# mcgill-cpslab/all-pairs-similarity

Hardware: AMD Instinct MI355X
Metric: scored candidate pairs/sec + achieved HBM GB/s, N=1M d=100k nnz=100, 1/2/4/8 GPU (higher is better)
Workload: dtype u16+f32

## Files before the change

### all-pairs-similarity_amd/csrc/apss_even.hpp

```cpp
#pragma once
#include <type_traits>
#include "apss_kernels.hpp"

namespace apss {

using ProbeArgsK = const __attribute__((address_space(4))) ProbeArgs;

template <int BLOCK, int U, int LONGCAP, bool SHARD, bool SIGNED, bool ACC8, bool MERGE, bool TWO = false>
__device__ __forceinline__ void probe_even_item(ProbeArgsK &a, const int tile, const int v0, const int v1, const bool own_tile, const bool first) {
  constexpr int NW = BLOCK / kWave;
  static_assert(NW == 8 || NW == 16, "8 or 16 waves");
  constexpr int NS = NW - 1;
  constexpr bool SLOT2 = BLOCK <= 512;
  constexpr uint32_t ABITS = ACC8 ? 8u : 16u;
  constexpr bool WIDE = ACC8 && BLOCK > 512;
  constexpr int CH = 16, LPC = CH / 2, GPW = kWave / LPC, WIN = GPW * U;
  constexpr int SLOTS = 2 * WIN < 48 ? 2 * WIN : (WIN > 48 ? WIN : 48);
  static_assert(SLOTS >= WIN, "the register window reads the first WIN slots of a strip");
  constexpr int GS = BLOCK > 512 ? SLOTS / GPW : ((SLOTS / GPW) + 1) & ~1;
  constexpr int SSZ = GPW * GS;
  static_assert(GPW == 8 && SLOTS % GPW == 0, "slot <-> (step, group) by shifts");
  constexpr int kLongLen = kLongLenW;
  constexpr int CBMAX = WIDE ? 131072 : (BLOCK <= 512 && !ACC8 ? 32768 : 65536);
  constexpr int APW = 32 / (int)ABITS;
  constexpr bool LEAN = !SIGNED;
  static_assert(1 + (NW - 1) * 2 * U < (1 << (ACC8 ? 8 : 16)), "the spare words' low accumulators must not wrap within a round");
  static_assert(!TWO || (BLOCK == 512 && ACC8 && !MERGE && !SIGNED && !SHARD), "two planes: the plain 512-thread kernel, 8-bit sums");
  __shared__ __attribute__((aligned(16))) uint32_t acc[CBMAX / APW + kWave];
  __shared__ __attribute__((aligned(16))) uint2 strips[3 * NS * SSZ + kWave];
  __shared__ uint2 longs[3 * LONGCAP];
  __shared__ float long_w[3 * LONGCAP];
  __shared__ uint2 facts[4];
  __shared__ unsigned long long stat[4];
  unsigned char *const smem_raw = reinterpret_cast<unsigned char *>(acc);
  uint32_t *const facts_w = reinterpret_cast<uint32_t *>(facts);

  int tid = threadIdx.x;
  asm volatile("" : "+v"(tid));
  const int wv = __builtin_amdgcn_readfirstlane(tid / kWave), ln = tid % kWave;
  const int cb = a.cb;
  const int F = a.flat_waves;
  const int A = NW - F;
  const int CAP = A * SLOTS;
  const uint32_t A8 = (uint32_t)A * (uint32_t)GPW;
  const float rcpA8 = 1.0f / (float)A8;
  const uint32_t magicA8 = 0xffffffffu / A8 + 1u;
  const int LOGG = a.flat_group_log2, G = 1 << LOGG;
  const uint32_t sub = (uint32_t)ln & (uint32_t)(G - 1);
  static_assert(!MERGE || SHARD, "merged rounds: term shards only");
  const int mlaunch = MERGE ? a.merge_log2 : 0;
  const int mlog = own_tile ? 0 : mlaunch;
  const int nv = own_tile ? a.nq_rows : a.nq;
  const int qtile = (v0 << mlog) / cb;
  const int64_t tile_row0 = (int64_t)tile * cb;
  const int unmerged_mark = own_tile ? kUnmergedBit : 0;
  const uint32_t lo = (uint32_t)(ln % LPC);
  const float cxs = a.cx_scale;

  const int64_t qbase = uniform_load(a.q_rowptr + (MERGE ? min(v0 << mlog, a.nq_rows) : v0)), qend = uniform_load(a.q_rowptr + (MERGE ? min(v1 << mlog, a.nq_rows) : v1));
  const int64_t pbase = uniform_load(a.tile_post_base + tile), pend = uniform_load(a.tile_post_base + tile + 1);
  const __amdgpu_buffer_rsrc_t rs_qi =
      __builtin_amdgcn_make_buffer_rsrc((void *)(a.q_idx + qbase), 0, (int)((qend - qbase) * 4), 0x00020000);
  const __amdgpu_buffer_rsrc_t rs_qv =
      __builtin_amdgcn_make_buffer_rsrc((void *)(a.q_val + qbase), 0, (int)((qend - qbase) * 4), 0x00020000);
  const __amdgpu_buffer_rsrc_t rs_tp = __builtin_amdgcn_make_buffer_rsrc(
      (void *)(a.tile_seg + (int64_t)tile * a.seg_stride), 0, (int)(a.seg_stride * 8), 0x00020000);
  const __amdgpu_buffer_rsrc_t rs_po =
      __builtin_amdgcn_make_buffer_rsrc((void *)(a.post_c + pbase), 0, (int)((pend - pbase) * 4), 0x00020000);
  constexpr uint32_t kOob = 0xfffffff0u;
  constexpr uint32_t kStale = 0x80000000u, kSwept = 0x40000000u;
  constexpr uint32_t kRare = 0x80000000u;
  constexpr uint32_t kCountMask = 0xffffu;
  constexpr int kFirstSkippable = BLOCK > 512 || !SHARD ? U - 1 : 0;

  if (first) {
    for (int i = tid * 4; i < cb / APW; i += BLOCK * 4) *reinterpret_cast<uint4 *>(acc + i) = make_uint4(0u, 0u, 0u, 0u);
    if constexpr (TWO)
      for (int i = tid * 4; i < cb / APW; i += BLOCK * 4) *reinterpret_cast<uint4 *>(acc + cb / APW + i) = make_uint4(0u, 0u, 0u, 0u);
  }
  if (tid < kWave) acc[CBMAX / APW + tid] = 1u;
  if (LEAN) {
    for (int i = tid; i < 3 * NS * SSZ; i += BLOCK) strips[i].x = kStale;
  }
  if (tid < 8) facts_w[tid] = 0;
  unsigned long long my_visits = 0;
  uint32_t my_cands = 0;
  uint32_t n_seen = 0;

  struct RowExt { int qb; int nnz; };
  struct TermW { uint32_t term; float w, qs; bool valid; };
  struct Seg { uint32_t s, len; float w; };
  struct WaveWork {
    uint32_t info;
    uint32_t flags;
    apss_u32x2 pc[U];
    float wq[U];
  };
  const int32_t *const rowptr_lo = reinterpret_cast<const int32_t *>(a.q_rowptr);
  const int qbase_lo = (int)(uint32_t)qbase;
  auto load_R = [&](int v) {
    RowExt r;
    const int row_a = min(v, nv - 1) << mlog, row_b = MERGE ? min(row_a + (1 << mlog), a.nq_rows) : row_a + 1;
    r.qb = rowptr_lo[2 * row_a];
    r.nnz = rowptr_lo[2 * row_b];
    return r;
  };
  auto load_I = [&](const RowExt &r, const int fi, const int v) {
    TermW t;
    const int kterm = ((fi * kWave) >> LOGG) + (ln >> LOGG);
    const int nnz = v < v1 ? r.nnz - r.qb : 0;
    t.valid = kterm < nnz;
    const uint32_t off = t.valid ? (uint32_t)(r.qb - qbase_lo + kterm) * 4u : kOob;
    t.term = __builtin_amdgcn_raw_buffer_load_b32(rs_qi, off, 0, 0);
    t.w = __uint_as_float(__builtin_amdgcn_raw_buffer_load_b32(rs_qv, off, 0, 0));
    t.qs = SHARD && !MERGE ? a.q_scale[min(v, nv - 1)] : 1.0f;
    return t;
  };
  auto load_P = [&](const TermW &t) {
    Seg g;
    const apss_u32x2 sg = __builtin_amdgcn_raw_buffer_load_b64(rs_tp, t.valid ? t.term * 8u : kOob, 0, 0);
    g.s = sg.x;
    g.len = sg.y;
    g.w = SHARD ? (t.qs > 0.f ? t.w * __builtin_amdgcn_rcpf(t.qs) : 0.f) : t.w;
    return g;
  };
  uint2 *const spare_item = strips + 3 * NS * SSZ + ln;
  auto flatten = [&](const Seg &g, const int ring, const int fs) {
    uint32_t len = g.len;
    my_visits += sub == 0u ? len : 0u;
    const bool is_long = len > (uint32_t)kLongLen;
    len = is_long ? 0u : len;
    const uint32_t nch = (len + CH - 1) / CH;
    const uint32_t mine = sub == 0u ? nch : 0u;
    const uint32_t incl = wave_incl_scan(mine);
    uint32_t base = 0;
    if (ln == kWave - 1) base = atomicAdd(&facts_w[2 * fs], incl);
    uint32_t j0 = (uint32_t)__builtin_amdgcn_readlane((int)base, kWave - 1) + incl - mine;
    if (LOGG == 2) j0 = (uint32_t)__builtin_amdgcn_update_dpp((int)j0, (int)j0, 0x00, 0xf, 0xf, false);
    else if (LOGG == 1) j0 = (uint32_t)__builtin_amdgcn_update_dpp((int)j0, (int)j0, 0xa0, 0xf, 0xf, false);
    const uint32_t wbits = __float_as_uint(cxs * g.w);
    uint2 *const st = strips + ring * (NS * SSZ);
    auto put = [&](const uint32_t k) {
      const uint32_t j = min(j0 + k, (uint32_t)CAP - 1u);
      const uint32_t u = (uint32_t)(((float)j + 0.5f) * rcpA8);
      const uint32_t r = j - u * A8;
      uint2 *const dst = k < nch ? st + (r >> 3) * SSZ + (r & 7u) * GS + u : spare_item;
      *dst = make_uint2((g.s + k * CH) * 4u, wbits);
    };
    const uint32_t two = LOGG == 2 ? 8u : (LOGG == 1 ? 6u : 3u);
    put(sub);
    put(sub + (uint32_t)G);
    if (LOGG < 2) put(sub + 2u * (uint32_t)G);
    const bool unfit = j0 + nch > (uint32_t)CAP;
    if (__any(is_long || unfit || nch > two)) {
      bool bad = unfit;
      if (is_long && sub == 0u) {
        const uint32_t k = atomicAdd(&facts_w[2 * fs + 1], 2u) >> 1;
        if (k < (uint32_t)LONGCAP) {
          longs[ring * LONGCAP + k] = make_uint2(g.s, g.len);
          long_w[ring * LONGCAP + k] = g.w;
        } else {
          bad = true;
        }
      }
      if (bad) atomicOr(&facts_w[2 * fs + 1], 1u);
      for (uint32_t k = two + sub; __any(k < nch); k += (uint32_t)G) put(k);
    }
  };
  struct StripRead { uint2 fc; uint2 it[U]; };
  auto strip_read = [&](StripRead &sr, const int ring, const int rank, const int fs) {
    sr.fc = facts[fs];
    const uint2 *const st = strips + (ring * NS + rank) * SSZ + (ln / LPC) * GS;
    if constexpr (GS % 2 == 0) {
#pragma unroll
      for (int u = 0; u + 1 < U; u += 2) {
        const uint4 two = *reinterpret_cast<const uint4 *>(st + u);
        sr.it[u] = make_uint2(two.x, two.y);
        sr.it[u + 1] = make_uint2(two.z, two.w);
      }
      if (U & 1) sr.it[U - 1] = st[U - 1];
    } else {
#pragma unroll
      for (int u = 0; u < U; ++u) sr.it[u] = st[u];
    }
    if (LEAN) {
      uint2 *const own = strips + (ring * NS + rank) * SSZ + (ln & 7) * GS + (ln >> 3);
      (ln < WIN ? own : spare_item)->x = kStale;
    }
  };
  auto strip_loads = [&](WaveWork &f, StripRead &sr, const int rank) {
    const uint32_t fx = (uint32_t)__builtin_amdgcn_readfirstlane((int)sr.fc.x), fy = (uint32_t)__builtin_amdgcn_readfirstlane((int)sr.fc.y);
    const uint32_t tot = (fy & 1u) ? 0u : fx;
    const uint32_t full = __umulhi(tot, magicA8);
    const int rem = (int)(tot - full * A8) - GPW * rank;
    const uint32_t mine = (uint32_t)GPW * full + (uint32_t)min(max(rem, 0), GPW);
    const bool rare = fy != 0u || tot > (uint32_t)(A * WIN);
    const uint32_t steps = min(full + (rem > 0 ? 1u : 0u), (uint32_t)U);
    f.info = mine | (rare ? kRare : 0u) | (steps << 16);
    f.flags = sr.fc.y;
#pragma unroll
    for (int u = 0; u < U; ++u) asm volatile("" : "+v"(sr.it[u].x), "+v"(sr.it[u].y));
    const uint32_t lane_off = lo * 8u + (LEAN && (fy & 1u) ? kSwept : 0u);
#pragma unroll
    for (int u = 0; u < U; ++u) {
      f.wq[u] = __uint_as_float(sr.it[u].y);
      const uint32_t off = LEAN ? sr.it[u].x + lane_off : ((uint32_t)(u * GPW + ln / LPC) < mine ? sr.it[u].x + lo * 8u : kOob);
      f.pc[u] = __builtin_amdgcn_raw_buffer_load_b64(rs_po, off, 0, 0);
    }
  };

  const bool stager = wv < F;
  const int rank = wv - F;
  WaveWork wfa, wfb;
  if constexpr (TWO) {
    wfb.info = 0u;
#pragma unroll
    for (int u = 0; u < U; ++u) wfb.pc[u] = apss_u32x2{0u, 0u};
  }
  constexpr int slack = 2;
  const int thr_c = (int)a.cx_theta - slack;
  const uint32_t thr1 = (uint32_t)max(thr_c, 1) - 1u;
  {
    const TermW I0 = load_I(load_R(v0), wv, v0), I1 = load_I(load_R(v0 + 1), wv, v0 + 1);
    const Seg P0 = load_P(I0), P1 = load_P(I1);
    __syncthreads();
    if (stager) {
      flatten(P0, 0, TWO ? 3 : 0);
      flatten(P1, 1, 1);
    }
    __syncthreads();
    if (!stager) {
      StripRead sr;
      strip_read(sr, 0, rank, TWO ? 3 : 0);
      strip_loads(wfa, sr, rank);
    }
  }

  if (stager) {
    RowExt R4 = load_R(v0 + 4);
    TermW Ic = load_I(load_R(v0 + 3), wv, v0 + 3);
    Seg Pc = load_P(load_I(load_R(v0 + 2), wv, v0 + 2));
    int r0 = 0;
    for (int v = v0; v < v1; ++v) {
      const int r2 = r0 == 0 ? 2 : r0 - 1;
      const RowExt R5 = load_R(v + 5);
      const TermW In = load_I(R4, wv, v + 4);
      const Seg Pn = load_P(Ic);
      flatten(Pc, r2, r2);
      if constexpr (TWO) {
        if (tid == 0) facts[r0] = make_uint2(0u, 0u);
        __syncthreads();
      } else {
        __syncthreads();
        if (tid == 0) facts[r0] = make_uint2(0u, 0u);
        __syncthreads();
      }
      R4 = R5;
      Ic = In;
      Pc = Pn;
      r0 = r0 == 2 ? 0 : r0 + 1;
    }
  } else {
    const int atid = tid - F * kWave, ABLOCK = A * kWave;
    auto clear_round = [&](const WaveWork &w, const uint32_t P) {
      *reinterpret_cast<uint32_t *>(smem_raw + (uint32_t)(CBMAX / APW) * 4u + (uint32_t)ln * 4u) = 0x0101u;
      if ((w.info & kRare) != 0u) {
        const uint32_t keep = P ? 0x00ff00ffu : 0xff00ff00u;
        for (int i = atid; i < cb / 2; i += ABLOCK) __hip_atomic_fetch_and(acc + i, keep, __ATOMIC_RELAXED, __HIP_MEMORY_SCOPE_WORKGROUP);
      } else {
        const int n = (int)((w.info >> 16) & 0xfu);
#pragma unroll
        for (int u = 0; u < U; ++u) {
          if (u >= kFirstSkippable && u >= n) break;
          smem_raw[(w.pc[u].x & 0xffffu) + P] = 0;
          smem_raw[(w.pc[u].y & 0xffffu) + P] = 0;
        }
      }
    };
    auto round = [&](auto plane, WaveWork &w0, WaveWork &w2, const int v, const int r0) {
      constexpr uint32_t P = TWO ? (uint32_t)decltype(plane)::value : 0u;
      const int r1 = r0 == 2 ? 0 : r0 + 1;
      const int q = v;
      auto report = [&](const bool cross, const uint32_t slot, const uint32_t sum) {
        bool ok = cross;
        if (ok && mlog == 0) ok = a.ext_id[tile_row0 + slot] != a.q_ext[q];
        const uint64_t o = wave_append(ok, &a.counters[kCtrResults]);
        if (ok && o < a.res_cap) {
          a.res_q[o] = q | unmerged_mark;
          a.res_c[o] = (int32_t)(tile_row0 + slot);
          a.res_s[o] = (float)sum / cxs;
        }
      };
      auto report_lane = [&](const uint32_t slot, const uint32_t sum) {
        if (mlog != 0 || a.ext_id[tile_row0 + slot] != a.q_ext[q]) {
          const uint64_t o = atomicAdd(&a.counters[kCtrResults], 1ull);
          if (o < a.res_cap) {
            a.res_q[o] = q | unmerged_mark;
            a.res_c[o] = (int32_t)(tile_row0 + slot);
            a.res_s[o] = (float)sum / cxs;
          }
        }
      };
      auto slot_of = [&](const uint32_t pcw) { return WIDE ? pcw >> 15 : (SLOT2 && (!ACC8 || TWO) ? (pcw & 0xffffu) >> 1 : pcw & 0xffffu); };
      auto prod = [&](const uint32_t pcw, const float wqs) {
        const float x = __builtin_fmaf(wqs, __half2float(__ushort_as_half((unsigned short)(WIDE ? pcw & 0x7fffu : pcw >> 16))), 1.0f);
        return SIGNED ? (uint32_t)max((int)x, 1) : (uint32_t)x;
      };
      auto half_of = [&](const uint32_t old_word, const uint32_t pcw) {
        if (WIDE) return __builtin_amdgcn_ubfe(old_word, (pcw >> 12) & 24u, 8u);
        if (TWO) return __builtin_amdgcn_ubfe(old_word, (pcw << 3) + 8u * P, 8u);
        return SLOT2 ? __builtin_amdgcn_ubfe(old_word, pcw << 3, ABITS) : (old_word >> ((pcw & 1u) << 4)) & 0xffffu;
      };
      constexpr int BATCH = 3;
      const uint32_t spare = (uint32_t)(CBMAX / APW) * 4u + (uint32_t)ln * 4u;
      auto add_or_spare = [&](const uint32_t pcw, const uint32_t p) -> uint32_t {
        if constexpr (TWO) {
          return atomicAdd(reinterpret_cast<uint32_t *>(smem_raw + (pcw ? pcw & 0xfffcu : spare)), p << (((pcw << 3) + 8u * P) & 31u));
        }
        const uint32_t addr = WIDE ? (pcw >> 15) & 0x1fffcu : (SLOT2 ? pcw & 0xfffcu : ((pcw & 0xffffu) >> 1) * 4u);
        const uint32_t sh = WIDE ? (pcw >> 12) & 24u : (SLOT2 ? (pcw << 3) & 31u : (pcw & 1u) << 4);
        return atomicAdd(reinterpret_cast<uint32_t *>(smem_raw + (pcw ? addr : spare)), p << sh);
      };
      auto visit2 = [&](const uint32_t x, const uint32_t y, const float wqs) {
        const uint32_t px = prod(x, wqs), py = prod(y, wqs);
        uint32_t ox = add_or_spare(x, LEAN && x == 0u ? 0u : px), oy = add_or_spare(y, LEAN && y == 0u ? 0u : py);
        ox = x ? half_of(ox, x) : thr1 + 1u;
        oy = y ? half_of(oy, y) : thr1 + 1u;
        my_cands += (ox == 0u ? 1u : 0u) + (oy == 0u ? 1u : 0u);
        if ((thr1 - ox < px) | (thr1 - oy < py)) {
          if (thr1 - ox < px) report_lane(slot_of(x), ox + px);
          if (thr1 - oy < py) report_lane(slot_of(y), oy + py);
        }
      };
      const int n_steps = (int)((w0.info >> 16) & 0xfu);
      if (LEAN) n_seen -= 2u * (uint32_t)max(n_steps, kFirstSkippable);
      auto issue_batch = [&](const int u0, uint32_t (&p0)[BATCH], uint32_t (&p1)[BATCH], uint32_t (&o0)[BATCH], uint32_t (&o1)[BATCH]) {
#pragma unroll
        for (int j = 0; j < BATCH; ++j) {
          const int u = u0 + j;
          if (u >= kFirstSkippable && u >= n_steps) break;
          if (u < U) {
            p0[j] = prod(w0.pc[u].x, w0.wq[u]);
            p1[j] = prod(w0.pc[u].y, w0.wq[u]);
            o0[j] = add_or_spare(w0.pc[u].x, p0[j]);
            o1[j] = add_or_spare(w0.pc[u].y, p1[j]);
          }
        }
      };
      auto check_batch = [&](const int u0, uint32_t (&p0)[BATCH], uint32_t (&p1)[BATCH], uint32_t (&o0)[BATCH], uint32_t (&o1)[BATCH]) {
        if constexpr (LEAN) {
          uint32_t top = 0;
#pragma unroll
          for (int j = 0; j < BATCH; ++j) {
            const int u = u0 + j;
            if (u >= kFirstSkippable && u >= n_steps) break;
            if (u < U) {
              o0[j] = half_of(o0[j], w0.pc[u].x);
              o1[j] = half_of(o1[j], w0.pc[u].y);
              uint32_t s0, s1;
              asm("v_min_u32 %0, 1, %1" : "=v"(s0) : "v"(o0[j]));
              asm("v_min_u32 %0, 1, %1" : "=v"(s1) : "v"(o1[j]));
              n_seen += s0 + s1;
              top = max(max(top, o0[j] + p0[j]), o1[j] + p1[j]);
            }
          }
          if (__any(top > thr1)) {
#pragma unroll
            for (int j = 0; j < BATCH; ++j) {
              const int u = u0 + j;
              if (u >= kFirstSkippable && u >= n_steps) break;
              if (u < U) {
                const uint32_t a0 = w0.pc[u].x ? o0[j] : thr1 + 1u, a1 = w0.pc[u].y ? o1[j] : thr1 + 1u;
                report(thr1 - a0 < p0[j], slot_of(w0.pc[u].x), a0 + p0[j]);
                report(thr1 - a1 < p1[j], slot_of(w0.pc[u].y), a1 + p1[j]);
              }
            }
          }
          return;
        }
        uint32_t n_cross = 0;
#pragma unroll
        for (int j = 0; j < BATCH; ++j) {
          const int u = u0 + j;
          if (u >= kFirstSkippable && u >= n_steps) break;
          if (u < U) {
            o0[j] = w0.pc[u].x ? half_of(o0[j], w0.pc[u].x) : thr1 + 1u;
            o1[j] = w0.pc[u].y ? half_of(o1[j], w0.pc[u].y) : thr1 + 1u;
            my_cands += (o0[j] == 0u ? 1u : 0u) + (o1[j] == 0u ? 1u : 0u);
            n_cross += (thr1 - o0[j] < p0[j] ? 1u : 0u) + (thr1 - o1[j] < p1[j] ? 1u : 0u);
          }
        }
        if (__any(n_cross != 0u)) {
#pragma unroll
          for (int j = 0; j < BATCH; ++j) {
            const int u = u0 + j;
            if (u >= kFirstSkippable && u >= n_steps) break;
            if (u < U) {
              report(thr1 - o0[j] < p0[j], slot_of(w0.pc[u].x), o0[j] + p0[j]);
              report(thr1 - o1[j] < p1[j], slot_of(w0.pc[u].y), o1[j] + p1[j]);
            }
          }
        }
      };
      if constexpr (TWO) clear_round(w2, P ^ 1u);
      StripRead sr;
      strip_read(sr, r1, rank, r1);
      {
        uint32_t p0[BATCH], p1[BATCH], o0[BATCH], o1[BATCH];
        issue_batch(0, p0, p1, o0, o1);
        asm volatile("" : "+v"(sr.fc.x), "+v"(sr.fc.y) : : "memory");
        __builtin_amdgcn_sched_barrier(0);
        strip_loads(w2, sr, rank);
        check_batch(0, p0, p1, o0, o1);
      }
#pragma unroll
      for (int u0 = BATCH; u0 < U; u0 += BATCH) {
        uint32_t p0[BATCH], p1[BATCH], o0[BATCH], o1[BATCH];
        issue_batch(u0, p0, p1, o0, o1);
        check_batch(u0, p0, p1, o0, o1);
      }
      const bool rare = (w0.info & kRare) != 0u;
      if (rare) {
        const uint32_t flags = (uint32_t)__builtin_amdgcn_readfirstlane((int)w0.flags);
        const int mc = (int)(w0.info & kCountMask);
        if (mc > WIN) {
          const uint2 *const st = strips + (r0 * NS + rank) * SSZ;
          for (int c0 = WIN; c0 < mc; c0 += GPW) {
            const int c = c0 + ln / LPC;
            const int cc = min(c, SLOTS - 1);
            const uint2 it = st[(cc & 7) * GS + (cc >> 3)];
            const apss_u32x2 two = __builtin_amdgcn_raw_buffer_load_b64(rs_po, c < mc ? it.x + lo * 8u : kOob, 0, 0);
            visit2(two.x, two.y, __uint_as_float(it.y));
          }
        }
        if (flags & 1u) {
          RowExt cur = load_R(v);
          cur.nnz -= cur.qb;
          cur.qb -= qbase_lo;
          const float qsv = SHARD && !MERGE ? uniform_load(a.q_scale + v) : 1.0f;
          const float iq = qsv > 0.f ? 1.0f / qsv : 0.f;
          for (int k = rank; k < cur.nnz; k += A) {
            const uint32_t off = (uint32_t)(cur.qb + k) * 4u;
            const uint32_t term = __builtin_amdgcn_raw_buffer_load_b32(rs_qi, off, 0, 0);
            const float wq_ = cxs * __uint_as_float(__builtin_amdgcn_raw_buffer_load_b32(rs_qv, off, 0, 0)) * iq;
            const apss_u32x2 sg = __builtin_amdgcn_raw_buffer_load_b64(rs_tp, term * 8u, 0, 0);
            for (uint32_t p = 2u * (uint32_t)ln; p < sg.y; p += 2u * kWave) {
              const apss_u32x2 two = __builtin_amdgcn_raw_buffer_load_b64(rs_po, (sg.x + p) * 4u, 0, 0);
              visit2(two.x, p + 1u < sg.y ? two.y : 0u, wq_);
            }
          }
        } else {
          const uint32_t n_long = min(flags >> 1, (uint32_t)LONGCAP);
          for (uint32_t j = 0; j < n_long; ++j) {
            const uint2 sgm = longs[r0 * LONGCAP + j];
            const float wq_ = cxs * long_w[r0 * LONGCAP + j];
            for (uint32_t k = 2u * (uint32_t)atid; k < sgm.y; k += 2u * (uint32_t)ABLOCK) {
              const apss_u32x2 a0 = __builtin_amdgcn_raw_buffer_load_b64(rs_po, (sgm.x + k) * 4u, 0, 0);
              visit2(a0.x, k + 1u < sgm.y ? a0.y : 0u, wq_);
            }
          }
        }
      }
      __syncthreads();
      if constexpr (TWO) return;

      if (LEAN) *reinterpret_cast<uint32_t *>(smem_raw + spare) = 1u;
      if (rare) {
        for (int i = atid * 4; i < cb / APW; i += ABLOCK * 4) *reinterpret_cast<uint4 *>(acc + i) = make_uint4(0u, 0u, 0u, 0u);
      } else {
        unsigned short *acc16w = reinterpret_cast<unsigned short *>(acc);
#pragma unroll
        for (int u = 0; u < U; ++u) {
          if (u >= kFirstSkippable && u >= n_steps) break;
          if (WIDE) {
            smem_raw[w0.pc[u].x >> 15] = 0;
            smem_raw[w0.pc[u].y >> 15] = 0;
          } else if (SLOT2 && ACC8) {
            smem_raw[w0.pc[u].x & 0xffffu] = 0;
            smem_raw[w0.pc[u].y & 0xffffu] = 0;
          } else if (SLOT2) {
            *reinterpret_cast<unsigned short *>(smem_raw + (w0.pc[u].x & 0xffffu)) = 0;
            *reinterpret_cast<unsigned short *>(smem_raw + (w0.pc[u].y & 0xffffu)) = 0;
          } else {
            acc16w[w0.pc[u].x & 0xffffu] = 0;
            acc16w[w0.pc[u].y & 0xffffu] = 0;
          }
        }
      }
      __syncthreads();
    };
    int r0 = 0;
    constexpr std::integral_constant<int, 0> even_round{};
    constexpr std::integral_constant<int, TWO ? 1 : 0> odd_round{};
    for (int v = v0; v < v1; v += 2) {
      round(even_round, wfa, wfb, v, r0);
      r0 = r0 == 2 ? 0 : r0 + 1;
      if (v + 1 >= v1) break;
      round(odd_round, wfb, wfa, v + 1, r0);
      r0 = r0 == 2 ? 0 : r0 + 1;
    }
    if constexpr (TWO) {
      if ((v1 - v0) & 1) clear_round(wfa, 0u);
      else clear_round(wfb, 1u);
    }
  }
  __syncthreads();
  if (tid < 3) stat[tid] = 0;
  __syncthreads();
  atomicAdd(&stat[0], my_visits);
  atomicAdd(&stat[1], (unsigned long long)(my_cands - n_seen));
  __syncthreads();
  if (tid == 0) {
    const unsigned long long twice = a.tri && tile < qtile ? 2ull : 1ull;
    atomicAdd(&a.counters[kCtrVisits], stat[0] * twice);
    atomicAdd(&a.counters[kCtrCands], stat[1] * twice);
    atomicAdd(&a.counters[kCtrDevVisits], stat[0]);
  }
}

template <int BLOCK, int U, int LONGCAP, bool SHARD, bool SIGNED, bool ACC8, bool MERGE, bool TWO = false>
__device__ __forceinline__ void probe_even_body(const ProbeArgs &a) {
  int g_tile = 0, g_v0 = 0, g_v1 = 0;
  if (!a.items) {
    const int cb = a.cb, mlaunch = MERGE ? a.merge_log2 : 0;
    const int tile = a.tile0 + blockIdx.x / a.n_chunks;
    const int c0 = (blockIdx.x % a.n_chunks) * a.q_chunk;
    const int row_lo = c0 << mlaunch, row_hi = MERGE ? min(a.nq_rows, (c0 + a.q_chunk) << mlaunch) : 0;
    const bool own_tile = mlaunch != 0 && a.q_slot_base >= 0 && (a.q_slot_base + row_lo) / cb <= tile && tile <= (a.q_slot_base + row_hi - 1) / cb;
    if (a.tri && tile > row_lo / cb) return;
    g_tile = tile | (own_tile ? kUnmergedBit : 0);
    g_v0 = own_tile ? row_lo : c0;
    g_v1 = own_tile ? row_hi : min(a.nq, c0 + a.q_chunk);
    asm volatile("" : "+s"(g_tile), "+s"(g_v0), "+s"(g_v1));
  }
  __shared__ int next_item;
  for (bool first = true;; first = false) {
    int tile, v0, v1;
    bool own_tile;
    if (a.items) {
      if (threadIdx.x == 0) next_item = (int)atomicAdd(a.work_ctr, 1ull);
      __syncthreads();
      const int idx = __builtin_amdgcn_readfirstlane(next_item);
      if (idx >= a.n_items) return;
      const ProbeItem *const it = a.items + idx;
      tile = uniform_load(&it->tile);
      v0 = uniform_load(&it->v0);
      v1 = uniform_load(&it->v1);
      own_tile = uniform_load(&it->own) != 0;
    } else {
      if (!first) return;
      tile = g_tile & ~kUnmergedBit;
      v0 = g_v0;
      v1 = g_v1;
      own_tile = (g_tile & kUnmergedBit) != 0;
    }
    ProbeArgsK *ak = reinterpret_cast<ProbeArgsK *>(reinterpret_cast<uintptr_t>(__builtin_amdgcn_kernarg_segment_ptr()));
    asm volatile("" : "+s"(ak));
    probe_even_item<BLOCK, U, LONGCAP, SHARD, SIGNED, ACC8, MERGE, TWO>(*ak, tile, v0, v1, own_tile, first);
  }
}

template <int BLOCK, int U, int LONGCAP, bool SHARD, bool SIGNED, bool ACC8>
__global__ __launch_bounds__(BLOCK, BLOCK <= 512 ? 2 * BLOCK / 256 : BLOCK / 256) void k_probe_even(const ProbeArgs a) {
  probe_even_body<BLOCK, U, LONGCAP, SHARD, SIGNED, ACC8, false>(a);
}

template <int U, bool ACC8>
__global__ __launch_bounds__(512, 4) void k_probe_even_merged(const ProbeArgs a) {
  probe_even_body<512, U, 128, true, false, ACC8, true>(a);
}

template <int U>
__global__ __launch_bounds__(512, 4) void k_probe_planes(const ProbeArgs a) {
  probe_even_body<512, U, 128, false, false, true, false, true>(a);
}

}
```

Before: 1081 billion.

## Wipe idle accumulator plane with bulk ds_write_addtid instead of per-candidate clears

For the two-plane 8-bit kernel with U>=5, the accumulator planes are split into separate 32 KB LDS regions. Each wave now zeros the idle plane wholesale using ds_write_addtid_b32 through M0 while it stages or scores the other plane. This replaces the scattered per-candidate byte clears and the atomic AND sweep on rare rounds. The trade is a fixed wipe cost proportional to the accumulator size every round, plus an lgkmcnt wait before each barrier, in exchange for fewer scattered LDS stores and simpler indexing.

```diff
diff --git a/all-pairs-similarity_amd/csrc/apss_even.hpp b/all-pairs-similarity_amd/csrc/apss_even.hpp
--- a/all-pairs-similarity_amd/csrc/apss_even.hpp
+++ b/all-pairs-similarity_amd/csrc/apss_even.hpp
@@ -26,6 +26,8 @@
   constexpr bool LEAN = !SIGNED;
   static_assert(1 + (NW - 1) * 2 * U < (1 << (ACC8 ? 8 : 16)), "the spare words' low accumulators must not wrap within a round");
   static_assert(!TWO || (BLOCK == 512 && ACC8 && !MERGE && !SIGNED && !SHARD), "two planes: the plain 512-thread kernel, 8-bit sums");
+  constexpr bool WIPE = TWO && U >= 5;
+  constexpr uint32_t kPlane = 32768u;
   __shared__ __attribute__((aligned(16))) uint32_t acc[CBMAX / APW + kWave];
   __shared__ __attribute__((aligned(16))) uint2 strips[3 * NS * SSZ + kWave];
   __shared__ uint2 longs[3 * LONGCAP];
@@ -76,7 +78,7 @@
   if (first) {
     for (int i = tid * 4; i < cb / APW; i += BLOCK * 4) *reinterpret_cast<uint4 *>(acc + i) = make_uint4(0u, 0u, 0u, 0u);
     if constexpr (TWO)
-      for (int i = tid * 4; i < cb / APW; i += BLOCK * 4) *reinterpret_cast<uint4 *>(acc + cb / APW + i) = make_uint4(0u, 0u, 0u, 0u);
+      for (int i = tid * 4; i < cb / APW; i += BLOCK * 4) *reinterpret_cast<uint4 *>(acc + (WIPE ? (int)kPlane / 4 : cb / APW) + i) = make_uint4(0u, 0u, 0u, 0u);
   }
   if (tid < kWave) acc[CBMAX / APW + tid] = 1u;
   if (LEAN) {
@@ -86,6 +88,37 @@
   unsigned long long my_visits = 0;
   uint32_t my_cands = 0;
   uint32_t n_seen = 0;
+
+  static_assert(!WIPE || sizeof(strips) + sizeof(longs) + sizeof(long_w) + sizeof(facts) + sizeof(stat) + 256  + 256 * (NW - 1) < 65536,
+                "M0[15:0] must hold the LDS address of acc + 256 wv wherever acc lies");
+  const int wipe_n = WIPE ? ((cb + 255) >> 8) - wv : 0;
+  const uint32_t wipe_m0 = (uint32_t)(uintptr_t)(__attribute__((address_space(3))) uint32_t *)acc + 256u * (uint32_t)wv;
+  auto wipe = [&](auto plane_c) {
+    constexpr int PL = (int)decltype(plane_c)::value * (int)kPlane;
+    uint32_t zero = 0u;
+    asm volatile("" : "+v"(zero));
+    uint32_t keep;
+    int n = wipe_n;
+    asm volatile("" : "+s"(n));
+#define APSS_WIPE_FOUR(JB)                                                                                                        \
+  if (32 * (JB) < n)                                                                                                              \
+    asm volatile("s_mov_b32 %0, m0\n\ts_mov_b32 m0, %2\n\ts_nop 0\n\t"                                                            \
+                 "ds_write_addtid_b32 %1 offset:%3\n\tds_write_addtid_b32 %1 offset:%4\n\t"                                      \
+                 "ds_write_addtid_b32 %1 offset:%5\n\tds_write_addtid_b32 %1 offset:%6\n\t"                                      \
+                 "s_mov_b32 m0, %0"                                                                                              \
+                 : "=&s"(keep)                                                                                                   \
+                 : "v"(zero), "s"(wipe_m0), "i"(PL + 8192 * (JB)), "i"(PL + 8192 * (JB) + 2048), "i"(PL + 8192 * (JB) + 4096),   \
+                   "i"(PL + 8192 * (JB) + 6144)                                                                                  \
+                 : "memory")
+    APSS_WIPE_FOUR(0);
+    APSS_WIPE_FOUR(1);
+    APSS_WIPE_FOUR(2);
+    APSS_WIPE_FOUR(3);
+#undef APSS_WIPE_FOUR
+  };
+  constexpr std::integral_constant<int, 0> plane0{};
+  constexpr std::integral_constant<int, 1> plane1{};
+  auto wipe_wait = [&] { asm volatile("s_waitcnt lgkmcnt(0)" : : : "memory"); };
 
   struct RowExt { int qb; int nnz; };
   struct TermW { uint32_t term; float w, qs; bool valid; };
@@ -241,14 +274,21 @@
     TermW Ic = load_I(load_R(v0 + 3), wv, v0 + 3);
     Seg Pc = load_P(load_I(load_R(v0 + 2), wv, v0 + 2));
     int r0 = 0;
+    uint32_t idle = kPlane;
     for (int v = v0; v < v1; ++v) {
       const int r2 = r0 == 0 ? 2 : r0 - 1;
       const RowExt R5 = load_R(v + 5);
       const TermW In = load_I(R4, wv, v + 4);
       const Seg Pn = load_P(Ic);
+      if constexpr (WIPE) {
+        if (idle) wipe(plane1);
+        else wipe(plane0);
+        idle ^= kPlane;
+      }
       flatten(Pc, r2, r2);
       if constexpr (TWO) {
         if (tid == 0) facts[r0] = make_uint2(0u, 0u);
+        if constexpr (WIPE) wipe_wait();
         __syncthreads();
       } else {
         __syncthreads();
@@ -264,6 +304,7 @@
     const int atid = tid - F * kWave, ABLOCK = A * kWave;
     auto clear_round = [&](const WaveWork &w, const uint32_t P) {
       *reinterpret_cast<uint32_t *>(smem_raw + (uint32_t)(CBMAX / APW) * 4u + (uint32_t)ln * 4u) = 0x0101u;
+      if constexpr (WIPE) return;
       if ((w.info & kRare) != 0u) {
         const uint32_t keep = P ? 0x00ff00ffu : 0xff00ff00u;
         for (int i = atid; i < cb / 2; i += ABLOCK) __hip_atomic_fetch_and(acc + i, keep, __ATOMIC_RELAXED, __HIP_MEMORY_SCOPE_WORKGROUP);
@@ -308,12 +349,17 @@
       };
       auto half_of = [&](const uint32_t old_word, const uint32_t pcw) {
         if (WIDE) return __builtin_amdgcn_ubfe(old_word, (pcw >> 12) & 24u, 8u);
+        if (WIPE) return __builtin_amdgcn_ubfe(old_word, pcw << 2, 8u);
         if (TWO) return __builtin_amdgcn_ubfe(old_word, (pcw << 3) + 8u * P, 8u);
         return SLOT2 ? __builtin_amdgcn_ubfe(old_word, pcw << 3, ABITS) : (old_word >> ((pcw & 1u) << 4)) & 0xffffu;
       };
       constexpr int BATCH = 3;
       const uint32_t spare = (uint32_t)(CBMAX / APW) * 4u + (uint32_t)ln * 4u;
       auto add_or_spare = [&](const uint32_t pcw, const uint32_t p) -> uint32_t {
+        if constexpr (WIPE) {
+          const uint32_t at = pcw ? (pcw >> 1) & 0x7ffcu : spare - kPlane * P;
+          return atomicAdd(reinterpret_cast<uint32_t *>(smem_raw + kPlane * P + at), p << ((pcw << 2) & 31u));
+        }
         if constexpr (TWO) {
           return atomicAdd(reinterpret_cast<uint32_t *>(smem_raw + (pcw ? pcw & 0xfffcu : spare)), p << (((pcw << 3) + 8u * P) & 31u));
         }
@@ -403,6 +449,7 @@
         }
       };
       if constexpr (TWO) clear_round(w2, P ^ 1u);
+      if constexpr (WIPE) wipe(std::integral_constant<int, (int)(P ^ 1u)>{});
       StripRead sr;
       strip_read(sr, r1, rank, r1);
       {
@@ -461,6 +508,7 @@
           }
         }
       }
+      if constexpr (WIPE) wipe_wait();
       __syncthreads();
       if constexpr (TWO) return;
 
@@ -499,10 +547,15 @@
       round(odd_round, wfb, wfa, v + 1, r0);
       r0 = r0 == 2 ? 0 : r0 + 1;
     }
-    if constexpr (TWO) {
+    if constexpr (TWO && !WIPE) {
       if ((v1 - v0) & 1) clear_round(wfa, 0u);
       else clear_round(wfb, 1u);
     }
+  }
+  if constexpr (WIPE) {
+    if ((v1 - v0) & 1) wipe(plane0);
+    else wipe(plane1);
+    wipe_wait();
   }
   __syncthreads();
   if (tid < 3) stat[tid] = 0;
```

Result: faster. 1108 billion (median of 6 runs) (+2.5%).
